# yangt1013/SPEINet

Hardware: AMD Instinct MI355X
Metric: deblurred 720p frames/sec (higher is better)
Workload: dtype f16 (correlation top2)

## Files before the change

include/speinet_hip.h:

```cpp
#ifndef SPEINET_HIP_H
#define SPEINET_HIP_H

#include <stdint.h>

#ifdef __cplusplus
extern "C" {
#endif

typedef void* spei_stream_t;

#define SPEI_ACT_NONE 0
#define SPEI_ACT_RELU 1
#define SPEI_ACT_GELU 2

#define SPEI_F32 0
#define SPEI_BF16 1
#define SPEI_F16 2

#define SPEI_CONV 0
#define SPEI_CONV_TRANSPOSED 1

int spei_version(void);
const char* spei_last_error(void);
const char* spei_arch(void);

int spei_any_nonzero(const float* x, int64_t n, int32_t* flag, spei_stream_t stream);

int spei_rl_prior(const float* img, float* out, float* scratch, int C, int H, int W, int iters, float lam,
                  spei_stream_t stream);

int spei_conv5_in(const float* img_chw, const float* w, const float* bias, float* out_hwc, int H, int W,
                  int Cout, spei_stream_t stream);

int spei_conv5_out(const float* in_hwc, int ldi, const float* w, const float* bias, float* out_chw, int H,
                   int W, int Cin, spei_stream_t stream);

int spei_igemm_f32(const float* a0, int lda0, int k0, const float* a1, int lda1, int k1, const float* w,
                   const float* bias, float* out, int ldo, const float* residual, int ldr,
                   const float* rowscale, int Hin, int Win, int Hout, int Wout, int N, int ksize, int stride,
                   int pad, int mode, int act, spei_stream_t stream);

int spei_igemm_f32_batched(const float* a0, int lda0, int k0, const float* a1, int lda1, int k1, const float* w,
                           const float* bias, float* out, int ldo, const float* residual, int ldr,
                           const float* rowscale, int Hin, int Win, int Hout, int Wout, int N, int ksize, int stride,
                           int pad, int mode, int act, int batch, spei_stream_t stream);

int spei_conv_slab16(int fmt, const void* a0, int lda0, int k0, const void* a1, int lda1, int k1, int a_fmt,
                     const void* wfrag_hi, const void* wfrag_lo, const float* bias, void* out, int ldo, int out_fmt,
                     const float* residual, int ldr, const float* rowscale, int Hin, int Win, int Hout, int Wout,
                     int N, int ksize, int stride, int pad, int act, int ln_input, spei_stream_t stream);

int spei_conv_slab16_batched(int fmt, const void* a0, int k0, int a_fmt, const void* wfrag, const void* wfrag_lo, const float* bias,
                             void* out, int out_fmt, const float* residual, int batch, int Hin, int Win, int Hout, int Wout, int N,
                             int ksize, int stride, int pad, int act, spei_stream_t stream);

int spei_conv32_ws16(int fmt, const void* a, int a_fmt, const void* wfrag, const float* bias, void* out, int out_fmt, int batch,
                     int H, int W, int act, spei_stream_t stream);

int spei_conv64_ws16(int fmt, const void* a, int a_fmt, const void* wfrag, const float* bias, void* out, int out_fmt, int batch,
                     int H, int W, int act, spei_stream_t stream);

int spei_mlp_fused16(int fmt, const float* x, float* out, const void* w1_frag, const float* b1, const void* w2_frag,
                     const float* b2, int64_t M, spei_stream_t stream);

int spei_convt2_slab16(int fmt, const void* a0, int lda0, int k0, int a_fmt, const void* wfrag00, const void* wfrag01,
// ... 365 lines not shown
```

speinet_amd/csrc/stencil.hip:

```cpp
#include <stdarg.h>
#include <string.h>
#include "common.h"

static thread_local char g_err[512] = "";
void spei_set_error(const char* fmt, ...) {
    va_list ap;
    va_start(ap, fmt);
    vsnprintf(g_err, sizeof(g_err), fmt, ap);
    va_end(ap);
}
extern "C" const char* spei_last_error(void) { return g_err; }
extern "C" int spei_version(void) { return 100; }
extern "C" const char* spei_arch(void) { return "gfx950"; }

__global__ void any_nonzero_kernel(const float* __restrict__ x, int64_t n, int32_t* flag) {
    int64_t i = (int64_t)blockIdx.x * blockDim.x + threadIdx.x;
    const int64_t step = (int64_t)gridDim.x * blockDim.x;
    bool nz = false;
    for (; i < n; i += step) nz |= (x[i] != 0.0f);
    if (__any(nz) && (threadIdx.x & 63) == 0) atomicOr(flag, 1);
}
extern "C" int spei_any_nonzero(const float* x, int64_t n, int32_t* flag, spei_stream_t stream) {
    SPEI_REQUIRE(x && flag && n > 0, "spei_any_nonzero: bad arguments");
    hipStream_t s = (hipStream_t)stream;
// ... 24 lines not shown
#pragma unroll
        for (int dy = 0; dy < 5; ++dy)
#pragma unroll
            for (int dx = 0; dx < 5; ++dx) b = fmaf(t[ly + dy][lx + dx], 0.04f, b);
        const float c0 = t[ly + 2][lx + 2];
        float lap = -t[ly + 1][lx + 2];
        lap -= t[ly + 2][lx + 1];
        lap = fmaf(4.0f, c0, lap);
        lap -= t[ly + 2][lx + 3];
        lap -= t[ly + 3][lx + 2];
        const float I = img[plane + (size_t)gy * W + gx];
        float c = I / b;
        if (c != c) c = 0.0f;
        if (c < 0.0f) c = 0.0f;
        out[plane + (size_t)gy * W + gx] = c * (c0 + lam * lap);
    }
}
extern "C" int spei_rl_prior(const float* img, float* out, float* scratch, int C, int H, int W, int iters, float lam,
                             spei_stream_t stream) {
    SPEI_REQUIRE(img && out && scratch && C > 0 && H > 0 && W > 0 && iters >= 1, "spei_rl_prior: bad arguments");
    SPEI_REQUIRE(out != img && scratch != img && out != scratch, "spei_rl_prior: buffers must be distinct");
    hipStream_t s = (hipStream_t)stream;
    dim3 grid(cdiv(W, RL_T), cdiv(H, RL_T), C);
    const float* src = img;
    for (int it = 0; it < iters; ++it) {
        float* dst = ((iters - 1 - it) % 2 == 0) ? out : scratch;
        hipLaunchKernelGGL(rl_iter_kernel, grid, dim3(256), 0, s, img, src, dst, H, W, lam);
        src = dst;
    }
    SPEI_CHECK_LAUNCH("spei_rl_prior");
    return 0;
}

constexpr int CI_TH = 8, CI_TW = 32, CI_P = CI_TW + 4 + 1;
__global__ __launch_bounds__(256) void conv5_in_kernel(const float* __restrict__ img, const float* __restrict__ w,
                                                       const float* __restrict__ bias, float* __restrict__ out,
                                                       int H, int W, int tiles_x, int ntiles) {
    __shared__ float tin[3 * (CI_TH + 4) * CI_P];
    const int tid = threadIdx.x, lane = tid & 63, wave = tid >> 6;
    const int fr = lane & 31, fk = lane >> 5;
    int koff[38];
    float bw[38];
#pragma unroll
    for (int kk = 0; kk < 38; ++kk) {
        const int k = 2 * kk + fk;
        const int t = k / 3, ci = k - 3 * t;
        const int dy = t / 5, dx = t - 5 * dy;
        koff[kk] = k < 75 ? (ci * (CI_TH + 4) + dy) * CI_P + dx : 0;
        bw[kk] = k < 75 ? w[(t * 32 + fr) * 3 + ci] : 0.0f;
    }
    const float bv = bias[fr];
    const float* a0 = tin + (wave * 2) * CI_P + fr;
    const int et = fr & 3, ecol = (fr >> 2) * 4;
    for (int tile = blockIdx.x; tile < ntiles; tile += gridDim.x) {
        const int ty = tile / tiles_x, tx = tile - ty * tiles_x;
        const int x0 = tx * CI_TW, y0 = ty * CI_TH;
        for (int i = tid; i < 3 * (CI_TH + 4) * (CI_TW + 4); i += 256) {
            const int c = i / ((CI_TH + 4) * (CI_TW + 4));
            const int r = i - c * (CI_TH + 4) * (CI_TW + 4);
            const int ly = r / (CI_TW + 4), lx = r - ly * (CI_TW + 4);
            const int gy = y0 + ly - 2, gx = x0 + lx - 2;
            tin[(c * (CI_TH + 4) + ly) * CI_P + lx] = (gy >= 0 && gy < H && gx >= 0 && gx < W) ? img[((size_t)c * H + gy) * W + gx] : 0.0f;
        }
        __syncthreads();
        float av[2][38];
#pragma unroll
// ... 5 lines not shown
        f32x16 acc[2];
#pragma unroll
        for (int i = 0; i < 2; ++i)
#pragma unroll
            for (int r = 0; r < 16; ++r) acc[i][r] = 0.f;
#pragma unroll
        for (int kk = 0; kk < 38; ++kk) {
            acc[0] = __builtin_amdgcn_mfma_f32_32x32x2f32(av[0][kk], bw[kk], acc[0], 0, 0, 0);
            acc[1] = __builtin_amdgcn_mfma_f32_32x32x2f32(av[1][kk], bw[kk], acc[1], 0, 0, 0);
        }
#pragma unroll
        for (int i = 0; i < 2; ++i) {
            const int gy = y0 + wave * 2 + i;
#pragma unroll
            for (int k = 0; k < 4; ++k) {
                float a[4];
#pragma unroll
                for (int e = 0; e < 4; ++e) a[e] = fmaxf(acc[i][4 * k + e] + bv, 0.f);
                quad_transpose4(a[0], a[1], a[2], a[3], et);
                const int gx = x0 + 8 * k + 4 * fk + et;
                if (gy < H && gx < W) *reinterpret_cast<f32x4*>(out + ((size_t)gy * W + gx) * 32 + ecol) = f32x4{a[0], a[1], a[2], a[3]};
            }
        }
    }
}
extern "C" int spei_conv5_in(const float* img_chw, const float* w, const float* bias, float* out_hwc, int H, int W,
                             int Cout, spei_stream_t stream) {
    SPEI_REQUIRE(img_chw && w && bias && out_hwc && H > 0 && W > 0, "spei_conv5_in: bad arguments");
    SPEI_REQUIRE(Cout == 32, "spei_conv5_in: Cout=%d (only n_feat=32 is built)", Cout);
    const int tiles_x = cdiv(W, CI_TW), ntiles = tiles_x * cdiv(H, CI_TH);
    hipLaunchKernelGGL(conv5_in_kernel, dim3(ntiles < 1024 ? ntiles : 1024), dim3(256), 0, (hipStream_t)stream,
                       img_chw, w, bias, out_hwc, H, W, tiles_x, ntiles);
    SPEI_CHECK_LAUNCH("spei_conv5_in");
    return 0;
}

constexpr int CO_TH = 8, CO_TW = 32, CO_P = 36;
__global__ __launch_bounds__(256) void conv5_out_kernel(const float* __restrict__ in, int ldi, const float* __restrict__ w,
                                                        const float* __restrict__ bias, float* __restrict__ out,
                                                        int H, int W) {
    extern __shared__ __attribute__((aligned(16))) float sm[];
    float* tin = sm;
    float* wl = sm + (CO_TH + 4) * (CO_TW + 4) * CO_P;
    const int x0 = blockIdx.x * CO_TW, y0 = blockIdx.y * CO_TH;
    for (int i = threadIdx.x; i < (CO_TH + 4) * (CO_TW + 4) * 8; i += 256) {
        const int pix = i >> 3, q = i & 7;
        const int ly = pix / (CO_TW + 4), lx = pix - ly * (CO_TW + 4);
        const int gy = y0 + ly - 2, gx = x0 + lx - 2;
        float4 v = make_float4(0.f, 0.f, 0.f, 0.f);
        if (gy >= 0 && gy < H && gx >= 0 && gx < W) v = *reinterpret_cast<const float4*>(in + ((size_t)gy * W + gx) * ldi + q * 4);
        *reinterpret_cast<float4*>(tin + pix * CO_P + q * 4) = v;
    }
    for (int i = threadIdx.x; i < 25 * 3 * 32; i += 256) {
        const int t = i / 96, r = i - t * 96, co = r / 32, ci = r - co * 32;
        wl[(co * 25 + t) * 32 + ci] = w[i];
    }
    __syncthreads();
    const int lx = threadIdx.x & 31, ly = threadIdx.x >> 5;
    const int gy = y0 + ly, gx = x0 + lx;
    float a0 = bias[0], a1 = bias[1], a2 = bias[2];
    for (int t = 0; t < 25; ++t) {
        const int dy = t / 5, dx = t - dy * 5;
        const float4* pin = reinterpret_cast<const float4*>(tin + ((ly + dy) * (CO_TW + 4) + lx + dx) * CO_P);
        const float4* w0 = reinterpret_cast<const float4*>(wl + (0 * 25 + t) * 32);
        const float4* w1 = reinterpret_cast<const float4*>(wl + (1 * 25 + t) * 32);
        const float4* w2 = reinterpret_cast<const float4*>(wl + (2 * 25 + t) * 32);
// ... 216 lines not shown
```

speinet_amd/engine.py:

```python
from __future__ import annotations

import contextlib
from functools import partial

import torch

from .ops import ACT_GELU, ACT_RELU, CONV_T, BMap, Ctx, FMap


def _resblocks(ctx: Ctx, f: FMap, blocks, extra=None, out=None) -> FMap:
    n = len(blocks)
    for i, pk in enumerate(blocks):
        last = i == n - 1
        f = ctx.resblock(f, pk, extra=extra if last else None, out=out if last else None)
    return f


def in_block(ctx: Ctx, frame: torch.Tensor, pk: dict) -> FMap:
    ctx = ctx.for_stage("enc")
    return _resblocks(ctx, ctx.conv5_in(frame, pk["head_w"], pk["head_b"]), pk["blocks"])


def enc_stage(ctx: Ctx, f: FMap, pk: dict, extra=None, out=None) -> FMap:
    ctx = ctx.for_stage("enc")
    n = pk["head_b"].numel()
    f = ctx.igemm(f, pk["head_w"], pk["head_b"], n, ksize=5, stride=2, act=ACT_RELU)
    return _resblocks(ctx, f, pk["blocks"], extra, out)


def enc(ctx: Ctx, frame: torch.Tensor, P: dict, extra=None, out=None) -> FMap:
    return enc_stage(ctx, enc_stage(ctx, in_block(ctx, frame, P["inBlock"]), P["encoder_first"]), P["encoder_second"], extra, out)


def enc_batched(ctx: Ctx, frames: list, P: dict, refs=None, sums=None):
    ctx = ctx.for_stage("enc")
    assert ctx.batched_available()
    if refs is not None:
        return _enc_batched_routed(ctx, frames, P, list(refs), list(sums))
    b, (h, w) = len(frames), frames[0].shape[-2:]
    ib = P["inBlock"]
    lv1 = BMap.empty(b, h, w, ib["head_b"].numel(), frames[0].device)
    lib_in = lambda i: ctx.conv5_in(frames[i], ib["head_w"], ib["head_b"], out=lv1.map(i))
    for i in range(b):
        lib_in(i)
    for pk in ib["blocks"]:
        lv1 = ctx.resblock_batched(lv1, pk)
    levels = [lv1]
    f = lv1
    for name in ("encoder_first", "encoder_second"):
        st = P[name]
        f = ctx.igemm_batched(f, st["head_w"], st["head_b"], st["head_b"].numel(), 5, stride=2, act=ACT_RELU)
        for pk in st["blocks"]:
            f = ctx.resblock_batched(f, pk)
        levels.append(f)
    return levels


def _enc_batched_routed(ctx: Ctx, frames: list, P: dict, refs: list, sums: list):
    b, (h, w) = len(frames), frames[0].shape[-2:]
    dev, idt = frames[0].device, ctx.inter_dtype()
    ib = P["inBlock"]
    f = BMap.empty(b, h, w, ib["head_b"].numel(), dev)
    for i in range(b):
        ctx.conv5_in(frames[i], ib["head_w"], ib["head_b"], out=f.map(i))
    levels = []
    for name in ("inBlock", "encoder_first", "encoder_second"):
        st = P[name]
        if name != "inBlock":
            f = ctx.igemm_batched(f, st["head_w"], st["head_b"], st["head_b"].numel(), 5, stride=2, act=ACT_RELU)
        for pk in st["blocks"][:-1]:
            f = ctx.resblock_batched(f, pk)
        keep = {r: FMap.empty(f.H, f.W, f.C, dev) for r in refs}
        if name != "encoder_second":
            nxt = BMap.empty(b, f.H, f.W, f.C, dev, idt)
            routes = [(i, None, keep.get(i), nxt.map(i)) for i in range(b)]
        else:
            nxt = None
            routes = [(i, j, dest, None) for i, j, dest in sums] + [(r, None, keep[r], None) for r in refs]
        ctx.resblock_batched(f, st["blocks"][-1], routes=routes)
        levels.append(keep)
        f = nxt
    return levels


def dec_stage(ctx: Ctx, f: FMap, pk: dict) -> FMap:
    f = _resblocks(ctx, f, pk["blocks"])
    return ctx.for_stage("convt").igemm(f, pk["tail_w"], pk["tail_b"], pk["tail_b"].numel(), ksize=3, stride=2, mode=CONV_T, act=ACT_RELU)


class SwinX:

    def __init__(self, ctx: Ctx, f_mid: FMap, sw: dict):
        ctx = ctx.for_stage("swin")
        self.f_mid = f_mid
        self.x_first = ctx.igemm(f_mid, sw["conv_first_w"], sw["conv_first_b"], 256, ksize=3)
        self.xt0 = ctx.layernorm(self.x_first.t, sw["pe_g"], sw["pe_b"])

# ... 197 lines not shown
            feat = y() if callable(y) else y
            if lane is not main:
                lane.wait_event(ready)
            swin(ctx, sx, feat, P["swin"], out=cat.view(128 * slot, 128))


def forward_sample(ctx: Ctx, x: torch.Tensor, P: dict, n_seq: int, has_ref: bool, out: torch.Tensor, sides=()) -> torch.Tensor:
    return _run(forward_sample_steps(ctx, x, P, n_seq, has_ref, out, sides), out)


def _run(steps, out):
    for plan in steps:
        plan.launch()
    return out


def forward_sample_steps(ctx: Ctx, x: torch.Tensor, P: dict, n_seq: int, has_ref: bool, out: torch.Tensor, sides=()):
    h, w = x.shape[-2:]
    h3, w3 = h // 4, w // 4
    dev = x.device
    lanes = _lanes(ctx, sides)
    if ctx.for_stage("enc").batched_available():
        yield from forward_batch_steps(ctx, x[None], P, n_seq, [not has_ref], out[None], sides)
        return
    multi = ctx.for_stage("swin").swin_multi_available()
    with _side_lanes(lanes):
        lv = None
        if has_ref:
            with torch.cuda.stream(lanes[-1]):
                lv = reference_pyramid(ctx, x[n_seq + 1], P)
        cat = FMap(torch.empty(h3 * w3, 128 * n_seq, device=dev), h3, w3, 128 * n_seq)
        mid = x[n_seq // 2]
        e0 = enc(ctx, mid, P)
        f_mid = enc(ctx, ctx.rl_prior(mid, 5, 0.01), P, extra=e0, out=cat.view(0, 128))
        others = [i for i in range(n_seq) if i != n_seq // 2]

        def neighbour(i, out=None):
            e = enc(ctx, x[i], P)
            return enc(ctx, ctx.rl_prior(x[i], 1, 0.01), P, extra=e, out=out)

        if multi:
            fb = BMap.empty(len(others), h3, w3, 128, dev)
            for k, i in enumerate(others):
                with torch.cuda.stream(lanes[k % len(lanes)]):
                    neighbour(i, fb.map(k))
        else:
            _swin_calls(ctx, f_mid, [partial(neighbour, i) for i in others], P, cat, lanes)
    if multi:
        yield from _fuse_tail(ctx, f_mid, fb, cat, lv, P, out, lanes)
    else:
        yield from _tail(ctx, cat, lv, P, out)


def forward_batch_steps(ctx: Ctx, x: torch.Tensor, P: dict, n_seq: int, zero_ref: list, out: torch.Tensor, sides=(), max_maps: int = 16):
    B = x.shape[0]
    h, w = x.shape[-2:]
    h3, w3 = h // 4, w // 4
    dev = x.device
    lanes = _lanes(ctx, sides)
    others = [i for i in range(n_seq) if i != n_seq // 2]
    b0 = 0
    while b0 < B:
        group, maps = [], 0
        while b0 + len(group) < B:
            need = 2 + 2 * len(others) + (0 if zero_ref[b0 + len(group)] else 1)
            if group and maps + need > max_maps:
                break
            group.append(b0 + len(group))
            maps += need
        frames, first = [], {}
        for b in group:
            first[b] = len(frames)
            mid = x[b, n_seq // 2]
            frames += [mid, ctx.rl_prior(mid, 5, 0.01)]
            for i in others:
                frames += [x[b, i], ctx.rl_prior(x[b, i], 1, 0.01)]
            if not zero_ref[b]:
                frames.append(x[b, n_seq + 1])
        if ctx.for_stage("enc").handoff16:
            cats, fbs, refs, sums = {}, {}, [], []
            for b in group:
                m0 = first[b]
                cats[b] = FMap(torch.empty(h3 * w3, 128 * n_seq, device=dev), h3, w3, 128 * n_seq)
                fbs[b] = BMap.empty(len(others), h3, w3, 128, dev)
                sums.append((m0 + 1, m0, cats[b].view(0, 128)))
                sums += [(m0 + 3 + 2 * k, m0 + 2 + 2 * k, fbs[b].map(k)) for k in range(len(others))]
                if not zero_ref[b]:
                    refs.append(m0 + 2 + 2 * len(others))
            r1, r2, r3 = enc_batched(ctx, frames, P, refs=refs, sums=sums)
            del frames
            for b in group:
                mr = first[b] + 2 + 2 * len(others)
                lv = None if zero_ref[b] else (r1[mr], r2[mr], r3[mr])
                yield from _fuse_tail(ctx, cats[b].view(0, 128), fbs[b], cats[b], lv, P, out[b], lanes)
            b0 += len(group)
            continue
        lv1, lv2, lv3 = enc_batched(ctx, frames, P)
        del frames
        for b in group:
            m0 = first[b]
            cat = FMap(torch.empty(h3 * w3, 128 * n_seq, device=dev), h3, w3, 128 * n_seq)
            f_mid = FMap(ctx.add(lv3.map(m0 + 1).t, lv3.map(m0).t), h3, w3, 128)
            cat.t[:, :128].copy_(f_mid.t)
            fb = BMap.empty(len(others), h3, w3, 128, dev)
            for k in range(len(others)):
                ctx.add(lv3.map(m0 + 3 + 2 * k).t, lv3.map(m0 + 2 + 2 * k).t, out=fb.map(k).t)
            mr = m0 + 2 + 2 * len(others)
            lv = None if zero_ref[b] else (lv1.map(mr), lv2.map(mr), lv3.map(mr))
            yield from _fuse_tail(ctx, f_mid, fb, cat, lv, P, out[b], lanes)
        b0 += len(group)


def _fuse_tail(ctx: Ctx, f_mid: FMap, fb: BMap, cat: FMap, lv, P: dict, out: torch.Tensor, lanes: list):
    if ctx.for_stage("swin").swin_multi_available():
        swin_multi(ctx, SwinX(ctx, f_mid, P["swin"]), fb, P["swin"], [cat.view(128 * slot, 128) for slot in range(1, fb.B + 1)])
    else:
        with _side_lanes(lanes, fork=False):
            _swin_calls(ctx, f_mid, [fb.map(k) for k in range(fb.B)], P, cat, lanes)
    yield from _tail(ctx, cat, lv, P, out)


def _tail(ctx: Ctx, cat: FMap, lv, P: dict, out: torch.Tensor):
    fw = P["fusion"]
    ff = ctx.igemm(cat, fw["w"], fw["b"], 128)
    plan = search_plan(ctx, ff, lv[2]) if lv is not None else self_plan(ctx, ff)
    yield plan
    if lv is not None:
        s, t3, t2, t1 = search_finish(ctx, plan, ff, *lv)
    else:
        s, t3, t2, t1 = self_finish(ctx, plan, ff, P)
    decode(ctx, ff, s, t3, t2, t1, P, out)


def encode_raw(ctx: Ctx, frame: torch.Tensor, P: dict) -> FMap:
    return enc(ctx, frame, P)


def encode_sum(ctx: Ctx, frame: torch.Tensor, iters: int, e_raw: FMap, P: dict) -> FMap:
    return enc(ctx, ctx.rl_prior(frame, iters, 0.01), P, extra=e_raw)


def reference_pyramid(ctx: Ctx, frame: torch.Tensor, P: dict):
    lv1 = in_block(ctx, frame, P["inBlock"])
    lv2 = enc_stage(ctx, lv1, P["encoder_first"])
    return lv1, lv2, enc_stage(ctx, lv2, P["encoder_second"])


def fuse_and_decode(ctx: Ctx, f_mid: FMap, feats: list, lv, P: dict, n_seq: int, out: torch.Tensor, sides=()) -> torch.Tensor:
    return _run(fuse_and_decode_steps(ctx, f_mid, feats, lv, P, n_seq, out, sides), out)


def fuse_and_decode_steps(ctx: Ctx, f_mid: FMap, feats: list, lv, P: dict, n_seq: int, out: torch.Tensor, sides=()):
    h3, w3 = f_mid.H, f_mid.W
    dev = f_mid.t.device
    lanes = _lanes(ctx, sides)
    cat = FMap(torch.empty(h3 * w3, 128 * n_seq, device=dev), h3, w3, 128 * n_seq)
    cat.t[:, :128].copy_(f_mid.t)
    fb = BMap(torch.cat([f.t for f in feats]), len(feats), h3, w3, 128)
    yield from _fuse_tail(ctx, f_mid, fb, cat, lv, P, out, lanes)


def forward_swint(ctx: Ctx, x: torch.Tensor, P: dict, n_seq: int, out: torch.Tensor, sides=()) -> torch.Tensor:
    h, w = x.shape[-2:]
    h3, w3 = h // 4, w // 4
    dev = x.device
    lanes = _lanes(ctx, sides if n_seq > 1 else ())
    with _side_lanes(lanes):
        cat = FMap(torch.empty(h3 * w3, 128 * n_seq, device=dev), h3, w3, 128 * n_seq)
        f_mid = enc(ctx, x[n_seq // 2], P, out=cat.view(0, 128))
        if n_seq == 1:
            f_trans = FMap.empty(h3, w3, 128, dev)
            swin(ctx, SwinX(ctx, f_mid, P["swin"]), f_mid, P["swin"], out=f_trans)
# ... 12 lines not shown
```

speinet_amd/ops.py:

```python
from __future__ import annotations

import ctypes as C
import dataclasses
from typing import Optional

import numpy as np
import torch

from . import _lib, y4m
from . import codec as _codec
from . import light as _light
from . import shake as _shake
from .pack import BF16, F16, F32, LP_DTYPE, PackedW, fmt_of

ACT_NONE, ACT_RELU, ACT_GELU = 0, 1, 2
CONV, CONV_T = 0, 1

PRECISIONS = ("f32", "bf16x3", "bf16", "f16")
CORR_PRECISIONS = ("bf16x3", "single", "top2")
_CORR_ALIASES = {"bf16": "single", "bf16r": "top2", "f16": "single"}


class FMap:
    __slots__ = ("t", "H", "W", "C", "ld", "off")
# ... 65 lines not shown

class _ApplyRoute(C.Structure):
    _fields_ = [("out32", C.c_void_p), ("out16", C.c_void_p), ("ld32", C.c_int32), ("src", C.c_int32), ("partner", C.c_int32),
                ("reserved", C.c_int32)]


class _timed:
    def __init__(self, ctx: "Ctx", name: str):
        self.on = ctx.profile is not None and name in ctx.profile
        self.ctx, self.name = ctx, name

    def __enter__(self):
        if self.on:
            self.s = torch.cuda.Event(enable_timing=True)
            self.e = torch.cuda.Event(enable_timing=True)
            self.s.record(torch.cuda.current_stream(self.ctx.device))
        return self

    def __exit__(self, *a):
        if self.on:
            self.e.record(torch.cuda.current_stream(self.ctx.device))
            self.ctx.profile[self.name].append((self.s, self.e))
        return False


def _tensor_bytes(x) -> int:
    t = x.t if hasattr(x, "t") else x
    return t.numel() * t.element_size() if torch.is_tensor(t) else 0


def _conv_sub(method: str, a, k, out):
    if method == "conv5_in":
        return "level1", 2.0 * 25 * 3 * 32 * a[0].shape[-2] * a[0].shape[-1], _tensor_bytes(a[0]) + _tensor_bytes(out)
    if method == "conv5_out":
        return "level1", 2.0 * 25 * 32 * 3 * a[0].H * a[0].W, _tensor_bytes(a[0]) + 12 * a[0].H * a[0].W
    src, n = a[0], a[3]
    ks = a[4] if len(a) > 4 else k.get("ksize", 1)
    if n == 32 and src.C == 32 and ks == 5 and k.get("stride", a[5] if len(a) > 5 else 1) == 1:
        maps = getattr(src, "B", 1)
        return "level1", 2.0 * 25 * 32 * 32 * maps * src.H * src.W, _tensor_bytes(src) + _tensor_bytes(out)
    return "rest", 0.0, 0


def _family(name: str):
    def deco(fn):
        def wrapper(self, *a, **k):
            pr = self.profile
            if pr is None or "families" not in pr:
                return fn(self, *a, **k)
            st = torch.cuda.current_stream(self.device)
            s_, e_ = torch.cuda.Event(enable_timing=True), torch.cuda.Event(enable_timing=True)
            s_.record(st)
            out = fn(self, *a, **k)
            e_.record(st)
            pr["families"].setdefault(name, []).append((s_, e_))
            if name == "conv":
                sub, fl, by = _conv_sub(fn.__name__, a, k, out)
                rec = pr.setdefault("conv_sub", {}).setdefault(sub, {"events": [], "flops": 0.0, "bytes": 0})
                rec["events"].append((s_, e_))
                rec["flops"] += fl
                rec["bytes"] += by
            return out
        wrapper.__name__, wrapper.__doc__ = fn.__name__, fn.__doc__
        return wrapper
    return deco

# ... 649 lines not shown
        assert gt.dtype == torch.float32 and gt.numel() == n_gt * 3 * patch * patch

        def put(what, pair, dtype):
            rec, rec_host = pair
            nr = (n_in + n_gt) * dtype.itemsize
            assert rec.device == self.device and rec.dtype == torch.uint8 and rec.numel() >= nr and not rec_host.is_cuda \
                and rec_host.dtype == torch.uint8 and rec_host.is_contiguous() and rec_host.numel() >= nr, what
            return pair

        infix, stages, _held = _stage_args(light, noise and (noise[:2], noise[2]), shake and (shake[:2], shake[2]), self.device, put)
        _lib.check(getattr(_lib.lib(), f"spei_train_batch_runs{infix}_u8")(self._tp(table), C.c_void_p(table_host.data_ptr()), n_in, n_gt, *stages,
                                                                          self._tp(input), self._tp(gt), patch, float(rgb_range), self._stream()),
                   f"spei_train_batch_runs{infix}_u8")

    def train_batch_codec(self, input: torch.Tensor, n_in: int, patch: int, rgb_range: float, records: torch.Tensor,
                          records_host: torch.Tensor, qtabs) -> None:
        nb = n_in * 16
        assert records.dtype == torch.uint8 and records.numel() >= nb and not records_host.is_cuda and records_host.dtype == torch.uint8 \
            and records_host.is_contiguous() and records_host.numel() >= nb
        assert input.dtype == torch.float32 and input.numel() == n_in * 3 * patch * patch
        q_dev, q_host, n_qtab = _qtabs(qtabs, self.device)
        _lib.check(_lib.lib().spei_train_batch_codec_f32(self._tp(input), n_in, patch, float(rgb_range), self._tp(records),
                                                         C.c_void_p(records_host.data_ptr()), self._tp(q_dev), C.c_void_p(q_host.data_ptr()), n_qtab,
                                                         self._stream()), "spei_train_batch_codec_f32")

    def rl_prior(self, img: torch.Tensor, iters: int, lam: float = 0.01) -> torch.Tensor:
        c, h, w = img.shape
        out = torch.empty_like(img)
        scratch = torch.empty_like(img)
        _lib.check(_lib.lib().spei_rl_prior(self._tp(img), self._tp(out), self._tp(scratch), c, h, w, iters, lam, self._stream()),
                   "spei_rl_prior")
        return out

    @_family("conv")
    def conv5_in(self, img: torch.Tensor, w: torch.Tensor, b: torch.Tensor, out: Optional[FMap] = None) -> FMap:
        c, h, wd = img.shape
        assert c == 3
        if out is None:
            out = FMap.empty(h, wd, b.numel(), img.device)
        assert (out.H, out.W, out.C, out.ld, out.off) == (h, wd, b.numel(), b.numel(), 0) and not out.lp
        _lib.check(_lib.lib().spei_conv5_in(self._tp(img), self._tp(w), self._tp(b), self._fp(out), h, wd, b.numel(), self._stream()),
                   "spei_conv5_in")
        return out

    @_family("conv")
    def conv5_out(self, f: FMap, w: torch.Tensor, b: torch.Tensor, out: torch.Tensor, w32=None,
                  b32: Optional[torch.Tensor] = None) -> torch.Tensor:
        assert out.shape == (3, f.H, f.W) and out.is_contiguous() and out.dtype == torch.float32
        if self.lp16 and w32 is not None and f.C == 32:
            _lib.check(_lib.lib().spei_conv5_out_slab16(self.fmt, self._fp(f), f.ld, f.fmt, self._tp(w32.frag(self.fmt)), self._tp(b32),
                                                       self._tp(out), f.H, f.W, self._stream()), "spei_conv5_out_slab16")
            return out
        if f.lp:
            f = FMap(f.t.float(), f.H, f.W, f.C, f.off)
        _lib.check(_lib.lib().spei_conv5_out(self._fp(f), f.ld, self._tp(w), self._tp(b), self._tp(out), f.H, f.W, f.C, self._stream()),
                   "spei_conv5_out")
        return out

    def _conv3_pipe_ok(self, a, w, N: int, ksize: int, stride: int, act: int, residual, out) -> bool:
        return (self.conv3_pipe and self.lp16 and ksize == 3 and stride == 1 and N == 256 and a.C == 256 and act == ACT_NONE
                and a.H % 6 == 0 and a.W % 16 == 0 and a.H * a.W <= (1 << 21) and a.t.dtype == torch.float32 and getattr(a, "ld", 256) == 256
                and getattr(a, "off", 0) == 0 and getattr(w, "fhi", None) is not None and tuple(w.shape) == (9, 256, 256)
                and (out is None or (out.t.dtype == torch.float32 and getattr(out, "ld", 256) == 256 and getattr(out, "off", 0) == 0
                                     and out.t.data_ptr() != a.t.data_ptr()))
                and (residual is None or (residual.t.dtype == torch.float32 and getattr(residual, "ld", 256) == 256 and getattr(residual, "off", 0) == 0)))

    def _persistent_conv(self, a, w, bias, N: int, ksize: int, stride: int, act: int, residual, out, batch: int) -> bool:
        tp, lib, f = self._tp, _lib.lib(), self.fmt
        if self._conv3_pipe_ok(a, w, N, ksize, stride, act, residual, out):
            _lib.check(lib.spei_conv3x3_256_pipe16(f, tp(a.t), tp(w.frag(f)), tp(bias), tp(residual.t) if residual is not None else _vp(0),
                                                   tp(out.t), batch, a.H, a.W, self._stream()), "spei_conv3x3_256_pipe16")
            return True
        if not (ksize == 5 and stride == 1 and a.C == N and residual is None and act in (ACT_NONE, ACT_RELU) and w.fhi is not None
                and (getattr(a, "ld", N), getattr(a, "off", 0), getattr(out, "ld", N), getattr(out, "off", 0)) == (N, 0, N, 0)
                and a.t.data_ptr() != out.t.data_ptr()):
# ... 362 lines not shown
```

speinet_amd/speinet.py:

```python
from __future__ import annotations

import inspect
import os
from types import SimpleNamespace
from typing import Optional, Sequence

import torch
import torch.nn as nn

from . import _lib, engine, ops, pack


class _BasicConv(nn.Module):
    def __init__(self, cin, cout, k, relu):
        super().__init__()
        layers = [nn.Conv2d(cin, cout, k, padding=k // 2)]
        if relu:
            layers.append(nn.ReLU(inplace=True))
        self.main = nn.Sequential(*layers)


class _SE(nn.Module):
    def __init__(self, c, reduction=4):
        super().__init__()
# ... 341 lines not shown
            d.t.copy_(f.t)
        g.replay()
        return s_out.clone()

    def _window_pieces_batched(self, ctx, x, keys, cache, zero_ref, P, tag, G, pf, used):
        from .ops import FMap
        h, w = x.shape[-2:]
        h3, w3 = h // 4, w // 4
        n, mid = self.n_sequence, self.n_sequence // 2
        plan, have = [], {}

        def lookup(key):
            if key in have:
                return have[key]
            hit = cache.get(key)
            if hit is not None:
                used.append(hit)
                have[key] = hit[0]
            return have.get(key)

        sums = [(mid, 5)] + [(i, 1) for i in range(n) if i != mid]
        for i, it in sums:
            if lookup((tag, keys[i], it)) is None:
                if lookup((tag, keys[i], "raw")) is None and not any(pk == (tag, keys[i], "raw") for pk, *_ in plan):
                    plan.append(((tag, keys[i], "raw"), i, 0, False))
                if not any(pk == (tag, keys[i], ("rl", it)) for pk, *_ in plan):
                    plan.append(((tag, keys[i], ("rl", it)), i, it, False))
        if not zero_ref and lookup((tag, keys[n + 1], "ref")) is None:
            plan.append(((tag, keys[n + 1], "ref"), n + 1, 0, True))
        if plan:
            sig = tuple((it, lv_) for _, _, it, lv_ in plan)

            def run(*fr):
                maps = [ctx.rl_prior(f, it, 0.01) if it else f for f, (_, _, it, _) in zip(fr, plan)]
                lv1, lv2, lv3 = engine.enc_batched(ctx, maps, P)
                outs = []
                for j, (_, _, _, levels) in enumerate(plan):
                    outs += [lv1.map(j), lv2.map(j), lv3.map(j)] if levels else [lv3.map(j)]
                return outs

            outs = iter(G(("pieces", sig, h, w), [x[0, i] for _, i, _, _ in plan], run))
            ev = torch.cuda.Event()
            made = {}
            for pk, _, _, levels in plan:
                made[pk] = tuple(next(outs) for _ in range(3)) if levels else next(outs)
            for i, it in sums:
                ks = (tag, keys[i], it)
                if ks not in have:
                    rl = made[(tag, keys[i], ("rl", it))]
                    raw = made.get((tag, keys[i], "raw"))
                    raw = raw if raw is not None else have[(tag, keys[i], "raw")]
                    made[ks] = FMap(ctx.add(rl.t, raw.t), h3, w3, 128)
            ev.record(pf)
            for pk, v in made.items():
                if not (isinstance(pk[2], tuple) and pk[2][0] == "rl"):
                    hit = cache.put(pk, (v, ev))
                    used.append(hit)
                    have[pk] = v
        f_mid = have[(tag, keys[mid], 5)]
        feats = [have[(tag, keys[i], 1)] for i in range(n) if i != mid]
        lv = None if zero_ref else have[(tag, keys[n + 1], "ref")]
        return f_mid, feats, lv

    GRAPH_LIMIT = 24

    def _trim_graphs(self) -> None:
        if len(self._graphs) >= self.GRAPH_LIMIT:
# ... 124 lines not shown
```

Baseline: 42.77.

## Fuse RL prior iterations per tile and batch conv5_in across frames

Adds a multi-job RL prior kernel that runs up to five iterations inside one launch, using shared-memory tiles with widened halos. Jobs for all frames go into one launch, replacing a launch plus a full-image global round trip per iteration. It also adds a persistent, double-buffered batched conv5_in kernel that processes all frames in one launch instead of one launch per frame. The cost is redundant halo computation, larger LDS use that may lower occupancy, and more complex indexing.

```diff
diff --git a/include/speinet_hip.h b/include/speinet_hip.h
--- a/include/speinet_hip.h
+++ b/include/speinet_hip.h
@@ -29,8 +29,14 @@
 int spei_rl_prior(const float* img, float* out, float* scratch, int C, int H, int W, int iters, float lam,
                   spei_stream_t stream);
 
+int spei_rl_prior_multi(const float* const* imgs, float* const* outs, float* const* scratch, const int* iters, int njobs, int C,
+                        int H, int W, float lam, spei_stream_t stream);
+
 int spei_conv5_in(const float* img_chw, const float* w, const float* bias, float* out_hwc, int H, int W,
                   int Cout, spei_stream_t stream);
+
+int spei_conv5_in_batched(const float* const* imgs_chw, int N, const float* w, const float* bias, float* out_nhwc, int H, int W,
+                          int Cout, spei_stream_t stream);
 
 int spei_conv5_out(const float* in_hwc, int ldi, const float* w, const float* bias, float* out_chw, int H,
                    int W, int Cin, spei_stream_t stream);
diff --git a/speinet_amd/csrc/stencil.hip b/speinet_amd/csrc/stencil.hip
--- a/speinet_amd/csrc/stencil.hip
+++ b/speinet_amd/csrc/stencil.hip
@@ -80,6 +80,202 @@
     return 0;
 }
 
+constexpr int RLM_T = 64, RLM_MAXN = 5, RLM_MAXJOBS = 8;
+struct RlJob {
+    const float* img;
+    const float* src;
+    float* dst;
+    int n;
+    int blk0;
+};
+struct RlJobTable {
+    RlJob job[RLM_MAXJOBS];
+    int njobs, nmax;
+    int fresh;
+    int H, W, tiles_x, tiles_per_plane;
+    float lam;
+};
+static inline size_t rlm_lds_bytes(int nmax, bool fresh) {
+    const size_t p = RLM_T + 4 * nmax;
+    const size_t x = fresh ? (nmax >= 3 ? p - 8 : 0) : p, y = nmax >= 2 ? p - 4 : 0;
+    return (p + y + x) * p * sizeof(float);
+}
+
+template <int J, int I>
+__device__ __forceinline__ float rl_px(const float (&r)[6][8], float img, float lam) {
+#pragma clang fp contract(off)
+    float b = 0.0f;
+#pragma unroll
+    for (int dy = 0; dy < 5; ++dy)
+#pragma unroll
+        for (int dx = 0; dx < 5; ++dx) b = __builtin_fmaf(r[J + dy][I + dx], 0.04f, b);
+    const float c0 = r[J + 2][I + 2];
+    float lap = -r[J + 1][I + 2];
+    lap -= r[J + 2][I + 1];
+    lap = __builtin_fmaf(4.0f, c0, lap);
+    lap -= r[J + 2][I + 3];
+    lap -= r[J + 3][I + 2];
+    float c = img / b;
+    if (c != c) c = 0.0f;
+    if (c < 0.0f) c = 0.0f;
+    return c * __builtin_fmaf(lam, lap, c0);
+}
+
+__global__ __launch_bounds__(256) void rl_multi_kernel(const RlJobTable tb) {
+    extern __shared__ __attribute__((aligned(16))) float rl_lds[];
+    const int tid = threadIdx.x, H = tb.H, W = tb.W;
+    const float lam = tb.lam;
+    const float* img = tb.job[0].img;
+    const float* src = tb.job[0].src;
+    float* dst = tb.job[0].dst;
+    int n = tb.job[0].n, blk = blockIdx.x;
+#pragma unroll
+    for (int j = 1; j < RLM_MAXJOBS; ++j)
+        if (j < tb.njobs && (int)blockIdx.x >= tb.job[j].blk0) {
+            img = tb.job[j].img, src = tb.job[j].src, dst = tb.job[j].dst, n = tb.job[j].n;
+            blk = blockIdx.x - tb.job[j].blk0;
+        }
+    const int pl = blk / tb.tiles_per_plane, tr = blk - pl * tb.tiles_per_plane;
+    const int ty = tr / tb.tiles_x, tx = tr - ty * tb.tiles_x;
+    const size_t plane = (size_t)pl * H * W;
+    const int P = RLM_T + 4 * tb.nmax;
+    float* const ib = rl_lds;
+    float* const bufY = ib + P * P;
+    float* const bufX = bufY + (tb.nmax >= 2 ? (P - 4) * P : 0);
+    const int S0 = RLM_T + 4 * n;
+    const int oy = ty * RLM_T - 2 * n, ox = tx * RLM_T - 2 * n;
+
+    auto stage = [&](const float* __restrict__ g, float* buf) {
+        const int fx = tid & 127, gx = ox + fx;
+        const bool col = gx >= 0 && gx < W;
+        const float* const gp = g + plane + min(max(gx, 0), W - 1);
+#pragma unroll
+        for (int j0 = 0; j0 < (RLM_T + 4 * RLM_MAXN) / 2; j0 += 14) {
+            if (2 * j0 >= S0) break;
+            float v[14];
+#pragma unroll
+            for (int j = 0; j < 14; ++j) {
+                const int gy = oy + (tid >> 7) + 2 * (j0 + j);
+                v[j] = gp[(size_t)min(max(gy, 0), H - 1) * W];
+            }
+#pragma unroll
+            for (int j = 0; j < 14; ++j) {
+                const int fy = (tid >> 7) + 2 * (j0 + j), gy = oy + fy;
+                if (fx < S0 && fy < S0) buf[fy * P + fx] = (col && gy >= 0 && gy < H) ? v[j] : 0.0f;
+            }
+        }
+    };
+    stage(img, ib);
+    if (!tb.fresh) stage(src, bufX);
+    __syncthreads();
+
+    for (int k = 1; k <= n; ++k) {
+        const int S = S0 - 4 * k;
+        const float* const in = (k & 1) ? (k == 1 && tb.fresh ? ib : bufX) : bufY;
+        float* const outl = (k & 1) ? bufY : bufX;
+        const int ly0 = oy + 2 * k, lx0 = ox + 2 * k;
+        const int io = 2 * k;
+        const int nstrips = S >> 2, nitems = nstrips * (S >> 1);
+        const int inv = 65536 / nstrips + 1;
+        for (int it = tid; it < nitems; it += 256) {
+            const int by = (it * inv) >> 16, bx = it - by * nstrips;
+            const int y = 2 * by, x = 4 * bx;
+            const int gy = ly0 + y, gx = lx0 + x;
+            float o[2][4] = {{0.0f, 0.0f, 0.0f, 0.0f}, {0.0f, 0.0f, 0.0f, 0.0f}};
+            if (gy + 1 >= 0 && gy < H && gx + 3 >= 0 && gx < W) {
+                float r[6][8];
+#pragma unroll
+                for (int j = 0; j < 6; ++j) {
+                    const f32x4 lo = *reinterpret_cast<const f32x4*>(in + (y + j) * P + x);
+                    const f32x4 hi = *reinterpret_cast<const f32x4*>(in + (y + j) * P + x + 4);
+#pragma unroll
+                    for (int e = 0; e < 4; ++e) r[j][e] = lo[e], r[j][4 + e] = hi[e];
+                }
+                float iv[2][4];
+#pragma unroll
+                for (int j = 0; j < 2; ++j) {
+                    const float2 a = *reinterpret_cast<const float2*>(ib + (y + j + io) * P + x + io);
+                    const float2 b = *reinterpret_cast<const float2*>(ib + (y + j + io) * P + x + io + 2);
+                    iv[j][0] = a.x, iv[j][1] = a.y, iv[j][2] = b.x, iv[j][3] = b.y;
+                }
+                o[0][0] = rl_px<0, 0>(r, iv[0][0], lam); o[0][1] = rl_px<0, 1>(r, iv[0][1], lam);
+                o[0][2] = rl_px<0, 2>(r, iv[0][2], lam); o[0][3] = rl_px<0, 3>(r, iv[0][3], lam);
+                o[1][0] = rl_px<1, 0>(r, iv[1][0], lam); o[1][1] = rl_px<1, 1>(r, iv[1][1], lam);
+                o[1][2] = rl_px<1, 2>(r, iv[1][2], lam); o[1][3] = rl_px<1, 3>(r, iv[1][3], lam);
+#pragma unroll
+                for (int j = 0; j < 2; ++j)
+#pragma unroll
+                    for (int i = 0; i < 4; ++i)
+                        if (gy + j < 0 || gy + j >= H || gx + i < 0 || gx + i >= W) o[j][i] = 0.0f;
+            }
+            if (k < n) {
+#pragma unroll
+                for (int j = 0; j < 2; ++j)
+                    *reinterpret_cast<f32x4*>(outl + (y + j) * P + x) = f32x4{o[j][0], o[j][1], o[j][2], o[j][3]};
+            } else {
+#pragma unroll
+                for (int j = 0; j < 2; ++j) {
+                    if (gy + j >= H) continue;
+                    float* const q = dst + plane + (size_t)(gy + j) * W + gx;
+                    if (gx + 3 < W && (reinterpret_cast<uintptr_t>(q) & 15) == 0) {
+                        *reinterpret_cast<f32x4*>(q) = f32x4{o[j][0], o[j][1], o[j][2], o[j][3]};
+                    } else {
+#pragma unroll
+                        for (int i = 0; i < 4; ++i)
+                            if (gx + i < W) q[i] = o[j][i];
+                    }
+                }
+            }
+        }
+        if (k < n) __syncthreads();
+    }
+}
+
+extern "C" int spei_rl_prior_multi(const float* const* imgs, float* const* outs, float* const* scratch, const int* iters,
+                                   int njobs, int C, int H, int W, float lam, spei_stream_t stream) {
+    SPEI_REQUIRE(imgs && outs && iters && njobs >= 1 && njobs <= RLM_MAXJOBS && C > 0 && H > 0 && W > 0,
+                 "spei_rl_prior_multi: bad arguments (1..%d jobs)", RLM_MAXJOBS);
+    int rounds = 0;
+    for (int j = 0; j < njobs; ++j) {
+        SPEI_REQUIRE(imgs[j] && outs[j] && iters[j] >= 1, "spei_rl_prior_multi: job %d: bad arguments", j);
+        float* const sc = scratch ? scratch[j] : nullptr;
+        SPEI_REQUIRE(iters[j] <= RLM_MAXN || sc, "spei_rl_prior_multi: job %d: %d iterations need a scratch image", j, iters[j]);
+        SPEI_REQUIRE(outs[j] != imgs[j] && sc != imgs[j] && sc != outs[j], "spei_rl_prior_multi: job %d: buffers must be distinct", j);
+        for (int i = 0; i < j; ++i)
+            SPEI_REQUIRE(outs[i] != outs[j] && outs[i] != imgs[j] && outs[j] != imgs[i] && (!sc || (sc != outs[i] && sc != imgs[i])),
+                         "spei_rl_prior_multi: jobs %d and %d: one job writes what the other reads or writes", i, j);
+        const int r = cdiv(iters[j], RLM_MAXN);
+        rounds = r > rounds ? r : rounds;
+    }
+    const int tiles_x = cdiv(W, RLM_T), tpp = tiles_x * cdiv(H, RLM_T);
+    SPEI_REQUIRE((int64_t)tpp * C * njobs < (int64_t)1 << 31, "spei_rl_prior_multi: too many tiles");
+    hipStream_t s = (hipStream_t)stream;
+    for (int r = 0; r < rounds; ++r) {
+        RlJobTable tb = {};
+        tb.H = H, tb.W = W, tb.tiles_x = tiles_x, tb.tiles_per_plane = tpp, tb.lam = lam;
+        for (int depth = RLM_MAXN; depth >= 1; --depth)
+            for (int j = 0; j < njobs; ++j) {
+                const int nr = cdiv(iters[j], RLM_MAXN), left = iters[j] - r * RLM_MAXN;
+                if (r >= nr || (left < RLM_MAXN ? left : RLM_MAXN) != depth) continue;
+                float* const at[2] = {outs[j], scratch ? scratch[j] : nullptr};
+                RlJob& q = tb.job[tb.njobs];
+                q.img = imgs[j];
+                q.src = r == 0 ? imgs[j] : at[(nr - r) & 1];
+                q.dst = at[(nr - 1 - r) & 1];
+                q.n = depth;
+                q.blk0 = tb.njobs * tpp * C;
+                tb.nmax = depth > tb.nmax ? depth : tb.nmax;
+                ++tb.njobs;
+            }
+        tb.fresh = r == 0;
+        const size_t lds = rlm_lds_bytes(tb.nmax, tb.fresh);
+        ensure_dyn_lds<rl_multi_kernel>(lds);
+        hipLaunchKernelGGL(rl_multi_kernel, dim3(tb.njobs * tpp * C), dim3(256), lds, s, tb);
+    }
+    SPEI_CHECK_LAUNCH("spei_rl_prior_multi");
+    return 0;
+}
+
 constexpr int CI_TH = 8, CI_TW = 32, CI_P = CI_TW + 4 + 1;
 __global__ __launch_bounds__(256) void conv5_in_kernel(const float* __restrict__ img, const float* __restrict__ w,
                                                        const float* __restrict__ bias, float* __restrict__ out,
@@ -151,6 +347,138 @@
     hipLaunchKernelGGL(conv5_in_kernel, dim3(ntiles < 1024 ? ntiles : 1024), dim3(256), 0, (hipStream_t)stream,
                        img_chw, w, bias, out_hwc, H, W, tiles_x, ntiles);
     SPEI_CHECK_LAUNCH("spei_conv5_in");
+    return 0;
+}
+
+constexpr int CI_NMAX = 16;
+constexpr int CI_NE = 3 * (CI_TH + 4) * (CI_TW + 4), CI_NST = (CI_NE + 255) / 256;
+constexpr int CI_TILE = 3 * (CI_TH + 4) * CI_P;
+struct Conv5InBatch {
+    const float* img[CI_NMAX];
+};
+__global__ __launch_bounds__(256) void conv5_in_batched_kernel(const Conv5InBatch tb, const float* __restrict__ w,
+                                                               const float* __restrict__ bias, float* __restrict__ out,
+                                                               int H, int W, int tiles_x, int ntiles, int total) {
+    __shared__ float tin[2][CI_TILE];
+    const int tid = threadIdx.x, lane = tid & 63, wave = tid >> 6;
+    const int fr = lane & 31, fk = lane >> 5;
+    int koff[38];
+    float bw[38];
+#pragma unroll
+    for (int kk = 0; kk < 38; ++kk) {
+        const int k = 2 * kk + fk;
+        const int t = k / 3, ci = k - 3 * t;
+        const int dy = t / 5, dx = t - 5 * dy;
+        koff[kk] = k < 75 ? (ci * (CI_TH + 4) + dy) * CI_P + dx : 0;
+        bw[kk] = k < 75 ? w[(t * 32 + fr) * 3 + ci] : 0.0f;
+    }
+    const float bv = bias[fr];
+    const int aoff = (wave * 2) * CI_P + fr;
+    const int et = fr & 3, ecol = (fr >> 2) * 4;
+    const int ly0 = tid / (CI_TW + 4), lx0 = tid - ly0 * (CI_TW + 4);
+    const size_t map_in = (size_t)H * W, map_out = (size_t)H * W * 32;
+
+    auto origin = [&](int t, int& m, int& y0, int& x0) {
+        m = t / ntiles;
+        const int r = t - m * ntiles, ty = r / tiles_x;
+        y0 = ty * CI_TH;
+        x0 = (r - ty * tiles_x) * CI_TW;
+    };
+    auto advance = [](int& c, int& ly, int& lx) {
+        lx += 256 % (CI_TW + 4);
+        ly += 256 / (CI_TW + 4);
+        if (lx >= CI_TW + 4) { lx -= CI_TW + 4; ++ly; }
+        if (ly >= CI_TH + 4) { ly -= CI_TH + 4; ++c; }
+    };
+    float sv[CI_NST];
+    auto load_tile = [&](int t) {
+        int m, y0, x0;
+        origin(t, m, y0, x0);
+        const float* im = tb.img[m];
+        int c = 0, ly = ly0, lx = lx0;
+#pragma unroll
+        for (int j = 0; j < CI_NST; ++j) {
+            const int cc = min(c, 2);
+            const int gy = min(max(y0 + ly - 2, 0), H - 1), gx = min(max(x0 + lx - 2, 0), W - 1);
+            sv[j] = im[cc * map_in + (size_t)gy * W + gx];
+            advance(c, ly, lx);
+        }
+    };
+    auto store_tile = [&](int t, int buf) {
+        int m, y0, x0;
+        origin(t, m, y0, x0);
+        int c = 0, ly = ly0, lx = lx0;
+#pragma unroll
+        for (int j = 0; j < CI_NST; ++j) {
+            const bool ok = ((unsigned)(y0 + ly - 2) < (unsigned)H) & ((unsigned)(x0 + lx - 2) < (unsigned)W);
+            if (c < 3) tin[buf][(c * (CI_TH + 4) + ly) * CI_P + lx] = ok ? sv[j] : 0.0f;
+            advance(c, ly, lx);
+        }
+    };
+
+    int t = blockIdx.x;
+    if (t >= total) return;
+    load_tile(t);
+    store_tile(t, 0);
+    lds_barrier();
+    int buf = 0;
+    for (; t < total; t += gridDim.x, buf ^= 1) {
+        const int tn = t + gridDim.x;
+        const int tl = tn < total ? tn : t;
+        load_tile(tl);
+        __builtin_amdgcn_sched_barrier(0);
+
+        const float* a0 = tin[buf] + aoff;
+        f32x16 acc[2];
+#pragma unroll
+        for (int i = 0; i < 2; ++i)
+#pragma unroll
+            for (int r = 0; r < 16; ++r) acc[i][r] = 0.f;
+#pragma unroll
+        for (int kk = 0; kk < 38; ++kk) {
+            const float av0 = a0[koff[kk]], av1 = a0[koff[kk] + CI_P];
+            acc[0] = __builtin_amdgcn_mfma_f32_32x32x2f32(av0, bw[kk], acc[0], 0, 0, 0);
+            acc[1] = __builtin_amdgcn_mfma_f32_32x32x2f32(av1, bw[kk], acc[1], 0, 0, 0);
+        }
+        __builtin_amdgcn_sched_barrier(0);
+        store_tile(tl, buf ^ 1);
+
+        int m, y0, x0;
+        origin(t, m, y0, x0);
+        float* const ob = out + (size_t)m * map_out;
+#pragma unroll
+        for (int i = 0; i < 2; ++i) {
+            const int gy = y0 + wave * 2 + i;
+#pragma unroll
+            for (int k = 0; k < 4; ++k) {
+                float a[4];
+#pragma unroll
+                for (int e = 0; e < 4; ++e) a[e] = fmaxf(acc[i][4 * k + e] + bv, 0.f);
+                quad_transpose4(a[0], a[1], a[2], a[3], et);
+                const int gx = x0 + 8 * k + 4 * fk + et;
+                if (gy < H && gx < W) *reinterpret_cast<f32x4*>(ob + ((size_t)gy * W + gx) * 32 + ecol) = f32x4{a[0], a[1], a[2], a[3]};
+            }
+        }
+        lds_barrier();
+    }
+}
+extern "C" int spei_conv5_in_batched(const float* const* imgs_chw, int N, const float* w, const float* bias, float* out_nhwc,
+                                     int H, int W, int Cout, spei_stream_t stream) {
+    SPEI_REQUIRE(imgs_chw && w && bias && out_nhwc && H > 0 && W > 0 && N >= 1 && N <= CI_NMAX,
+                 "spei_conv5_in_batched: bad arguments (1..%d images)", CI_NMAX);
+    SPEI_REQUIRE(Cout == 32, "spei_conv5_in_batched: Cout=%d (only n_feat=32 is built)", Cout);
+    Conv5InBatch tb = {};
+    for (int i = 0; i < N; ++i) {
+        SPEI_REQUIRE(imgs_chw[i], "spei_conv5_in_batched: image %d is NULL", i);
+        tb.img[i] = imgs_chw[i];
+    }
+    const int tiles_x = cdiv(W, CI_TW), ntiles = tiles_x * cdiv(H, CI_TH);
+    SPEI_REQUIRE((int64_t)ntiles * N < (int64_t)1 << 31, "spei_conv5_in_batched: too many tiles");
+    const int total = ntiles * N;
+    const int grid = 3 * spei_num_cus();
+    hipLaunchKernelGGL(conv5_in_batched_kernel, dim3(total < grid ? total : grid), dim3(256), 0, (hipStream_t)stream,
+                       tb, w, bias, out_nhwc, H, W, tiles_x, ntiles, total);
+    SPEI_CHECK_LAUNCH("spei_conv5_in_batched");
     return 0;
 }
 
diff --git a/speinet_amd/engine.py b/speinet_amd/engine.py
--- a/speinet_amd/engine.py
+++ b/speinet_amd/engine.py
@@ -40,9 +40,7 @@
     b, (h, w) = len(frames), frames[0].shape[-2:]
     ib = P["inBlock"]
     lv1 = BMap.empty(b, h, w, ib["head_b"].numel(), frames[0].device)
-    lib_in = lambda i: ctx.conv5_in(frames[i], ib["head_w"], ib["head_b"], out=lv1.map(i))
-    for i in range(b):
-        lib_in(i)
+    ctx.conv5_in_batched(frames, ib["head_w"], ib["head_b"], lv1)
     for pk in ib["blocks"]:
         lv1 = ctx.resblock_batched(lv1, pk)
     levels = [lv1]
@@ -61,8 +59,7 @@
     dev, idt = frames[0].device, ctx.inter_dtype()
     ib = P["inBlock"]
     f = BMap.empty(b, h, w, ib["head_b"].numel(), dev)
-    for i in range(b):
-        ctx.conv5_in(frames[i], ib["head_w"], ib["head_b"], out=f.map(i))
+    ctx.conv5_in_batched(frames, ib["head_w"], ib["head_b"], f)
     levels = []
     for name in ("inBlock", "encoder_first", "encoder_second"):
         st = P[name]
@@ -326,12 +323,12 @@
         cat = FMap(torch.empty(h3 * w3, 128 * n_seq, device=dev), h3, w3, 128 * n_seq)
         mid = x[n_seq // 2]
         e0 = enc(ctx, mid, P)
-        f_mid = enc(ctx, ctx.rl_prior(mid, 5, 0.01), P, extra=e0, out=cat.view(0, 128))
+        f_mid = enc(ctx, ctx.rl_prior_multi([(mid, 5)], 0.01)[0], P, extra=e0, out=cat.view(0, 128))
         others = [i for i in range(n_seq) if i != n_seq // 2]
 
         def neighbour(i, out=None):
             e = enc(ctx, x[i], P)
-            return enc(ctx, ctx.rl_prior(x[i], 1, 0.01), P, extra=e, out=out)
+            return enc(ctx, ctx.rl_prior_multi([(x[i], 1)], 0.01)[0], P, extra=e, out=out)
 
         if multi:
             fb = BMap.empty(len(others), h3, w3, 128, dev)
@@ -365,10 +362,10 @@
         frames, first = [], {}
         for b in group:
             first[b] = len(frames)
-            mid = x[b, n_seq // 2]
-            frames += [mid, ctx.rl_prior(mid, 5, 0.01)]
-            for i in others:
-                frames += [x[b, i], ctx.rl_prior(x[b, i], 1, 0.01)]
+            rl = ctx.rl_prior_multi([(x[b, n_seq // 2], 5)] + [(x[b, i], 1) for i in others], 0.01)
+            frames += [x[b, n_seq // 2], rl[0]]
+            for k, i in enumerate(others):
+                frames += [x[b, i], rl[1 + k]]
             if not zero_ref[b]:
                 frames.append(x[b, n_seq + 1])
         if ctx.for_stage("enc").handoff16:
@@ -431,7 +428,7 @@
 
 
 def encode_sum(ctx: Ctx, frame: torch.Tensor, iters: int, e_raw: FMap, P: dict) -> FMap:
-    return enc(ctx, ctx.rl_prior(frame, iters, 0.01), P, extra=e_raw)
+    return enc(ctx, ctx.rl_prior_multi([(frame, iters)], 0.01)[0], P, extra=e_raw)
 
 
 def reference_pyramid(ctx: Ctx, frame: torch.Tensor, P: dict):
diff --git a/speinet_amd/ops.py b/speinet_amd/ops.py
--- a/speinet_amd/ops.py
+++ b/speinet_amd/ops.py
@@ -121,6 +121,8 @@
 def _conv_sub(method: str, a, k, out):
     if method == "conv5_in":
         return "level1", 2.0 * 25 * 3 * 32 * a[0].shape[-2] * a[0].shape[-1], _tensor_bytes(a[0]) + _tensor_bytes(out)
+    if method == "conv5_in_batched":
+        return "level1", 2.0 * 25 * 3 * 32 * len(a[0]) * a[0][0].shape[-2] * a[0][0].shape[-1], sum(_tensor_bytes(x) for x in a[0]) + _tensor_bytes(out)
     if method == "conv5_out":
         return "level1", 2.0 * 25 * 32 * 3 * a[0].H * a[0].W, _tensor_bytes(a[0]) + 12 * a[0].H * a[0].W
     src, n = a[0], a[3]
@@ -836,6 +838,22 @@
                    "spei_rl_prior")
         return out
 
+    RL_MAX_JOBS, RL_FUSED_ITERS = 8, 5
+
+    def rl_prior_multi(self, jobs, lam: float = 0.01) -> list:
+        jobs = list(jobs)
+        c, h, w = jobs[0][0].shape
+        assert all(img.shape == (c, h, w) and img.dtype == torch.float32 for img, _ in jobs)
+        outs = [torch.empty_like(img) for img, _ in jobs]
+        for g in range(0, len(jobs), self.RL_MAX_JOBS):
+            grp, n = jobs[g:g + self.RL_MAX_JOBS], len(jobs[g:g + self.RL_MAX_JOBS])
+            scratch = [torch.empty_like(img) if it > self.RL_FUSED_ITERS else None for img, it in grp]
+            ptrs = lambda ts: (C.c_void_p * n)(*[self._tp(t) for t in ts])
+            _lib.check(_lib.lib().spei_rl_prior_multi(ptrs([img for img, _ in grp]), ptrs(outs[g:g + n]), ptrs(scratch),
+                                                      (C.c_int * n)(*[it for _, it in grp]), n, c, h, w, lam, self._stream()),
+                       "spei_rl_prior_multi")
+        return outs
+
     @_family("conv")
     def conv5_in(self, img: torch.Tensor, w: torch.Tensor, b: torch.Tensor, out: Optional[FMap] = None) -> FMap:
         c, h, wd = img.shape
@@ -845,6 +863,20 @@
         assert (out.H, out.W, out.C, out.ld, out.off) == (h, wd, b.numel(), b.numel(), 0) and not out.lp
         _lib.check(_lib.lib().spei_conv5_in(self._tp(img), self._tp(w), self._tp(b), self._fp(out), h, wd, b.numel(), self._stream()),
                    "spei_conv5_in")
+        return out
+
+    CONV5_IN_MAX = 16
+
+    @_family("conv")
+    def conv5_in_batched(self, imgs: list, w: torch.Tensor, b: torch.Tensor, out: BMap) -> BMap:
+        c, h, wd = imgs[0].shape
+        assert c == 3 and all(x.shape == (3, h, wd) and x.dtype == torch.float32 for x in imgs)
+        assert (out.B, out.H, out.W, out.C) == (len(imgs), h, wd, b.numel()) and out.t.dtype == torch.float32
+        for g in range(0, len(imgs), self.CONV5_IN_MAX):
+            grp = imgs[g:g + self.CONV5_IN_MAX]
+            ptrs = (C.c_void_p * len(grp))(*[self._tp(x) for x in grp])
+            _lib.check(_lib.lib().spei_conv5_in_batched(ptrs, len(grp), self._tp(w), self._tp(b), self._fp(out.map(g)), h, wd, b.numel(),
+                                                        self._stream()), "spei_conv5_in_batched")
         return out
 
     @_family("conv")
diff --git a/speinet_amd/speinet.py b/speinet_amd/speinet.py
--- a/speinet_amd/speinet.py
+++ b/speinet_amd/speinet.py
@@ -397,7 +397,8 @@
             sig = tuple((it, lv_) for _, _, it, lv_ in plan)
 
             def run(*fr):
-                maps = [ctx.rl_prior(f, it, 0.01) if it else f for f, (_, _, it, _) in zip(fr, plan)]
+                rl = iter(ctx.rl_prior_multi([(f, it) for f, (_, _, it, _) in zip(fr, plan) if it], 0.01) if any(it for _, _, it, _ in plan) else ())
+                maps = [next(rl) if it else f for f, (_, _, it, _) in zip(fr, plan)]
                 lv1, lv2, lv3 = engine.enc_batched(ctx, maps, P)
                 outs = []
                 for j, (_, _, _, levels) in enumerate(plan):
```

Result: no change. 42.94, median of 6 (+0.4%).
